# saumyarr8/ApproximateQueryEngine

Hardware: AMD Instinct MI355X
Metric: aggregates/sec (10M-row-per-GPU APPROX AVG/SUM/COUNT with 95% CI, CLT --e 0.01) + achieved HBM GB/s (higher is better)
Workload: dtype f64; 1 GPU; configs[1]: 10M-row APPROX AVG/SUM/COUNT, CLT --e 0.01 percent (never converges: full 20% dual-pointer sweep, should_stop armed), table resident in HBM; step = 100 launches x 32 different queries per launch, every result fetched; rows_per_gpu=10000000, global_rows=10000000, queries_per_launch=32, samples_per_query_per_gpu=4000000

## Files before the change

approximatequeryengine_amd/csrc/kernels.hpp:

```cpp
#pragma once

#include <hip/hip_runtime.h>

#include <cstdint>

#include "../../include/aqe_hip.h"
#include "planner.hpp"

namespace aqe {

constexpr int kBlockThreads = 256;
constexpr int kWavesPerBlock = kBlockThreads / 64;
constexpr int kTileUnroll = 8;
constexpr int kTileOrdinals = 64 * kTileUnroll;
constexpr int kDenseTileOrdinals = 2 * kTileOrdinals;
__host__ __device__ inline bool is_dense16(uint64_t step, uint32_t flags, uint64_t seg_len) { return step == 1 && !(flags & AQE_F_PAIR) && seg_len >= static_cast<uint64_t>(kTileOrdinals); }
inline uint64_t tile_ordinals(uint64_t step, uint32_t flags, uint64_t seg_len) { return is_dense16(step, flags, seg_len) ? kDenseTileOrdinals : kTileOrdinals; }
constexpr uint32_t kFamLinear = 1u << 8;
constexpr int kMaxBlocks = 2048;
constexpr unsigned kRoundGridCap = 1024;
constexpr int kVec = AQE_MOMENT_VEC;
constexpr int kShards = 64;
constexpr int kShardStride = 32;
constexpr int kCounterWords = (kShards + 1) * kShardStride;
// ... 186 lines not shown
    LeanTail tail;
    LeanRuns runs;
};
static_assert(sizeof(LeanLaunch) <= 4096, "kernel arguments are limited to 4 KB");
constexpr int kUnionMaxPieces = 512;
constexpr int kUnionMaxEntries = 768;
constexpr int kUnionMaxIncidences = 2048;
constexpr int kUnionMaxRows = 256;
constexpr int kUnionWgPieces = 32;
constexpr int kUnionJudgeSlots = 32;
constexpr int kUnionDenseWaves = 4;
constexpr int kUnionMaxTilesPerWg = 64 * kPersistWaves;
constexpr uint32_t kUnionTileWhole = 1u << 31;
struct LeanUnion {
    const uint64_t* piece_lo;
    const uint64_t* piece_hi;
    const uint32_t* piece_entry;
    const uint32_t* target_begin;
    const uint32_t* target_entry;
    uint32_t npieces, ntargets, nincidences, nentries;
    uint32_t pad[2];
};
static_assert(sizeof(LeanUnion) == 64, "the union header is staged as 8 words");
hipError_t launch_sweep_lean(const LeanLaunch& a, unsigned grid, bool nt, hipStream_t s, hipEvent_t ev0 = nullptr, hipEvent_t ev1 = nullptr);
hipError_t launch_sweep_lean_multi(const LeanLaunch* table, const unsigned long long* wg_map, unsigned long long epoch, unsigned grid, bool nt,
                                   hipStream_t s, hipEvent_t ev0 = nullptr, hipEvent_t ev1 = nullptr);

hipError_t launch_replay(const double* totals, uint32_t rounds, uint32_t has_topup, const FoldParams& fp,
                         const FinalizeParams& fin, QueryState* state, aqe_result* result, hipStream_t s);

struct ReplayItem {
    uint32_t rounds, has_topup;
    FoldParams fp;
    FinalizeParams fin;
    QueryState* state;
    aqe_result* result;
};
hipError_t launch_replay_batch(const ReplayItem* items, uint32_t n, const double* totals, uint64_t row_stride, hipStream_t s);

hipError_t launch_round(const RoundLaunch& a, hipStream_t s, hipEvent_t ev0 = nullptr, hipEvent_t ev1 = nullptr);
hipError_t launch_indexed(const RoundLaunch& a, const uint64_t* idx, uint64_t n_idx, hipStream_t s, hipEvent_t ev0 = nullptr,
                          hipEvent_t ev1 = nullptr);
hipError_t launch_permuted(const RoundLaunch& a, const PermSpec& perm, uint64_t shard_lo, uint64_t shard_rows, hipStream_t s, hipEvent_t ev0 = nullptr,
                           hipEvent_t ev1 = nullptr);
hipError_t launch_gather_permuted(const aqe_record* aos, const PermSpec& perm, aqe_record* out, hipStream_t s);
hipError_t launch_update(QueryState* state, const double* vec, const FoldParams& p, int reset_state, hipStream_t s);
hipError_t launch_finalize(const QueryState* state, const FinalizeParams& p, aqe_result* out, hipStream_t s);

hipError_t launch_gather(const aqe_record* aos, uint64_t shard_lo, const DevFamily* fams, uint32_t nfam,
// ... 49 lines not shown
```

approximatequeryengine_amd/csrc/lean.hip:

```cpp
#include <hip/hip_ext.h>

#include "device_common.hpp"

namespace aqe {
namespace {

#define AQE_RLX __ATOMIC_RELAXED, __HIP_MEMORY_SCOPE_AGENT

typedef const AQE_KARG LeanLaunch* LeanKarg;

#ifdef AQE_LEAN_STAMPS
#if AQE_LEAN_STAMPS + 0 >= 2
#define LEAN_STAMP_BLOCKS 2
#define LEAN_STAMP_BASE (static_cast<size_t>(epoch & 1ull) * kLeanStampWords)
#else
#define LEAN_STAMP_BLOCKS 1
#define LEAN_STAMP_BASE static_cast<size_t>(0)
#endif
constexpr size_t kLeanStampWords = (static_cast<size_t>(kMaxPersistGrid) * kPersistWaves + 1 + kPersistWaves) * 8;
__device__ unsigned long long g_lean_stamps[LEAN_STAMP_BLOCKS * kLeanStampWords];
#define LEAN_STAMP(slot) do { if (lane == 0 && blockIdx.x < static_cast<unsigned>(kMaxPersistGrid)) g_lean_stamps[LEAN_STAMP_BASE + (static_cast<size_t>(blockIdx.x) * kPersistWaves + wave) * 8 + (slot)] = __builtin_amdgcn_s_memrealtime(); } while (0)
#define LEAN_STAMP_FOLD(slot) do { if (threadIdx.x == 0) g_lean_stamps[LEAN_STAMP_BASE + static_cast<size_t>(kMaxPersistGrid) * kPersistWaves * 8 + (slot)] = __builtin_amdgcn_s_memrealtime(); } while (0)
#define LEAN_STAMP_JUDGE(slot) do { if (lane == 0) g_lean_stamps[LEAN_STAMP_BASE + (static_cast<size_t>(kMaxPersistGrid) * kPersistWaves + 1 + wave) * 8 + (slot)] = __builtin_amdgcn_s_memrealtime(); } while (0)
#define LEAN_STAMP_HWID(slot) do { if (lane == 0) g_lean_stamps[LEAN_STAMP_BASE + (static_cast<size_t>(kMaxPersistGrid) * kPersistWaves + 1 + wave) * 8 + (slot)] = __builtin_amdgcn_s_getreg((31 << 11) | 4); } while (0)
#else
#define LEAN_STAMP(slot) do { } while (0)
#define LEAN_STAMP_FOLD(slot) do { } while (0)
#define LEAN_STAMP_JUDGE(slot) do { } while (0)
#endif

__device__ __forceinline__ void lean_state_store(QueryState* g, const QueryState& st) {
    static_assert(sizeof(QueryState) % 8 == 0, "state is moved as 8-byte words");
    const unsigned long long* s = reinterpret_cast<const unsigned long long*>(&st);
    unsigned long long* d = reinterpret_cast<unsigned long long*>(g);
#pragma unroll
    for (unsigned i = 0; i < sizeof(QueryState) / 8; ++i) __hip_atomic_store(d + i, s[i], AQE_RLX);
}

__device__ __forceinline__ u64 read_lane_u64(u64 v, unsigned src_lane) {
    const unsigned lo = __builtin_amdgcn_readlane(static_cast<unsigned>(v), src_lane);
    const unsigned hi = __builtin_amdgcn_readlane(static_cast<unsigned>(v >> 32), src_lane);
    return (static_cast<u64>(hi) << 32) | lo;
}

__device__ __forceinline__ u64* lean_t0_word(unsigned* counter) { return reinterpret_cast<u64*>(counter + kShards * kShardStride + 8); }

struct __attribute__((packed, aligned(8))) Row2 { double x, y; };

template <bool kNT>
__device__ __forceinline__ void lean_tile(const double* base, unsigned rem, const double* safe, int lane, int has_where, double wmin, double wmax,
                                          double shift, TileAcc& ta) {
    Row2 v2[kTileUnroll];
    if (rem >= static_cast<unsigned>(kDenseTileOrdinals)) {
        const Row2* const p = reinterpret_cast<const Row2*>(base) + lane;
#pragma unroll
        for (int k = 0; k < kTileUnroll; ++k) {
            if (kNT) {
                v2[k].x = __builtin_nontemporal_load(&p[k * 64].x);
                v2[k].y = __builtin_nontemporal_load(&p[k * 64].y);
            } else {
                v2[k] = p[k * 64];
            }
        }
        ta.nv = 2u * kTileUnroll;
        if (has_where) {
#pragma unroll
            for (int k = 0; k < kTileUnroll; ++k) {
                const double x = v2[k].x, y = v2[k].y;
                const bool px = x >= wmin && x <= wmax, py = y >= wmin && y <= wmax;
                const double dx = px ? x - shift : 0.0, dy = py ? y - shift : 0.0;
// ... 214 lines not shown
            auto below = [&](double v, unsigned by) { return kW >= 16 || q >= by ? v : 0.0; };
            double p = tot[cc];
            p += below(dpp_f64<0x111>(p), 1u);
            p += below(dpp_f64<0x112>(p), 2u);
            p += below(dpp_f64<0x114>(p), 4u);
            if constexpr (kW >= 16) p += dpp_f64<0x118>(p);
            if constexpr (kW == 32) {
                const double carry = __shfl(p, static_cast<int>((static_cast<unsigned>(lane) & 32u) | 15u), 64);
                p += (lane & 16) ? carry : 0.0;
            }
            tot[cc] = p;
        }
        lean_judge<kW>(Tm, tot, static_cast<unsigned>(lane), 0ull, epoch, lds_res);
        wave_lds_handoff();
#ifdef AQE_LEAN_STAMPS
        if (m0 == wave * kPer) { LEAN_STAMP_JUDGE(0); LEAN_STAMP_HWID(2); }
#endif
        if constexpr (kW == 32) lean_send_result<32>(Tm, lds_res, static_cast<unsigned>(lane));
        else lean_send_result<kW>(*reinterpret_cast<const LeanTail*>(my_tails), results + slot0 * kLeanResWords, static_cast<unsigned>(lane));
        LEAN_STAMP_JUDGE(1);
    }
}

template <bool kNT>
__device__ __forceinline__ void lean_union(const LeanLaunch& a, const LeanUnion* const U, const LeanLaunch* const members, const unsigned nmem,
                                           const unsigned bid, const unsigned G, const unsigned long long epoch,
                                           double (&lds_part)[kMaxPersistRounds][kPersistWaves][kVec], double (&lds_round)[kMaxPersistRounds][kVec],
                                           unsigned (&lds_mask)[kPersistWaves], int& s_last) {
    static_assert(kUnionWgPieces <= kMaxPersistRounds && kUnionWgPieces <= 32, "a share's pieces: a row of lds_part and a mask bit each");
    static_assert(sizeof(LeanUnion) + sizeof(unsigned) <= sizeof(lds_round), "the union's header is staged in lds_round, the largest round count after it");
    unsigned* const lds_max_rounds = reinterpret_cast<unsigned*>(&lds_round[0][0]) + sizeof(LeanUnion) / sizeof(unsigned);
    const int lane = threadIdx.x & 63;
    const unsigned wave = threadIdx.x >> 6;
    const unsigned t_lo = bid * a.tiles_per_wg;
    const unsigned t_end = t_lo + a.tiles_per_wg < a.ntiles ? t_lo + a.tiles_per_wg : a.ntiles;
    const u64* const tile_row = reinterpret_cast<const u64*>(U + 1);
    const unsigned* const tile_meta = reinterpret_cast<const unsigned*>(tile_row + a.ntiles);
    const unsigned* const wg = tile_meta + ((a.ntiles + 1u) & ~1u) + static_cast<size_t>(bid) * (kUnionWgPieces + 1);
    const unsigned my_t = t_lo + wave + kPersistWaves * static_cast<unsigned>(lane);
    u64 my_row = 0;
    unsigned my_meta = 0;
    if (my_t < t_end) { my_row = tile_row[my_t]; my_meta = tile_meta[my_t]; }
    const unsigned p0 = __builtin_amdgcn_readfirstlane(wg[0]);
    unsigned my_entry = 0;
    if (wave == 0 && lane < kUnionWgPieces) my_entry = wg[1 + lane];
#ifdef AQE_LEAN_STAMPS
    asm volatile("s_waitcnt vmcnt(0)" ::: "memory");
    LEAN_STAMP(1);
#endif
    const bool head_stager = wave == kPersistWaves - 2u;
    u64 head_word = 0;
    if (head_stager && static_cast<unsigned>(lane) < sizeof(LeanUnion) / 8u) head_word = reinterpret_cast<const u64*>(U)[lane];
#pragma unroll
    for (unsigned i = 0; i < kMaxPersistRounds * kVec / 64; ++i) {
        const unsigned x = static_cast<unsigned>(lane) + 64u * i;
        lds_part[x >> 3][wave][x & 7u] = 0.0;
    }

    double ps = 0.0, pq = 0.0;
    unsigned pn = 0, pv = 0, cur = ~0u, touched = 0;
    auto take = [&](unsigned piece, const TileAcc& ta) {
        if (piece != cur) {
            if (cur != ~0u) {
                const double v[7] = {static_cast<double>(pn), ps, pq, static_cast<double>(pv), 0.0, 0.0, 0.0};
                const double mine = wave_sum7(v, lane);
                if ((lane & 7) == 0 && lane < 32) lds_part[cur - p0][wave][lane >> 3] = mine;
                touched |= 1u << (cur - p0);
                ps = 0.0; pq = 0.0; pn = 0; pv = 0;
            }
            cur = piece;
        }
        pn += ta.n; pv += ta.nv; ps += ta.s; pq += ta.q;
    };
    for (unsigned j = 0;; ++j) {
        if (t_lo + wave + kPersistWaves * j >= t_end) break;
        const u64 row = read_lane_u64(my_row, j);
        const unsigned meta = __builtin_amdgcn_readlane(my_meta, j), piece = meta & 0xffffu;
        const double* const base = a.amount + row;
        if (meta & kUnionTileWhole) {
            TileAcc ta;
            lean_tile<kNT>(base, static_cast<unsigned>(kDenseTileOrdinals), a.amount, lane, a.has_where, a.wmin, a.wmax, a.shift, ta);
            take(piece, ta);
#ifdef AQE_LEAN_STAMPS
            if (j == 0) LEAN_STAMP(2);
#endif
            continue;
        }
        const unsigned vhi = (meta >> 16) & 0x7ffu, vlo = (meta >> 27) & 1u;
        Row2 v2[kTileUnroll];
        bool ok[kTileUnroll];
#pragma unroll
        for (int k = 0; k < kTileUnroll; ++k) {
            const unsigned oi = 2u * static_cast<unsigned>(lane) + 128u * static_cast<unsigned>(k);
            ok[k] = oi + 1u < vhi;
            const Row2* const p = reinterpret_cast<const Row2*>(ok[k] ? base + oi : a.amount);
            if (kNT) {
                v2[k].x = __builtin_nontemporal_load(&p->x);
                v2[k].y = __builtin_nontemporal_load(&p->y);
            } else {
                v2[k] = *p;
            }
        }
        const double xo = (vhi & 1u) ? base[vhi - 1u] : 0.0;
        const u64 phi = U->piece_hi[piece];
        const bool two = phi - row < vhi;
        const unsigned mid = two ? static_cast<unsigned>(phi - row) : vhi;
        const unsigned hi = two ? (U->piece_hi[piece + 1u] - row < vhi ? static_cast<unsigned>(U->piece_hi[piece + 1u] - row) : vhi) : vhi;
        TileAcc t0, t1;
        auto add = [&](double x, unsigned r, bool ld) {
            const bool i0 = ld && r >= vlo && r < mid, i1 = ld && r >= mid && r < hi;
            const bool w = !a.has_where || (x >= a.wmin && x <= a.wmax);
            const double d0 = i0 && w ? x - a.shift : 0.0, d1 = i1 && w ? x - a.shift : 0.0;
            t0.nv += i0 ? 1u : 0u; t0.n += i0 && w ? 1u : 0u; t0.s += d0; t0.q += d0 * d0;
            t1.nv += i1 ? 1u : 0u; t1.n += i1 && w ? 1u : 0u; t1.s += d1; t1.q += d1 * d1;
        };
#pragma unroll
        for (int k = 0; k < kTileUnroll; ++k) {
            const unsigned oi = 2u * static_cast<unsigned>(lane) + 128u * static_cast<unsigned>(k);
            add(v2[k].x, oi, ok[k]);
            add(v2[k].y, oi + 1u, ok[k]);
        }
        if (vhi & 1u) add(xo, vhi - 1u, lane == 0);
        take(piece, t0);
        if (two) take(piece + 1u, t1);
#ifdef AQE_LEAN_STAMPS
        if (j == 0) LEAN_STAMP(2);
#endif
    }
    LEAN_STAMP(3);
    if (cur != ~0u) take(~0u, TileAcc{});
    if (lane == 0) lds_mask[wave] = touched;
    if (head_stager && static_cast<unsigned>(lane) < sizeof(LeanUnion) / 8u) reinterpret_cast<u64*>(&lds_round[0][0])[lane] = head_word;
    if (head_stager && lane == 0) *lds_max_rounds = 0u;
    __syncthreads();

    if (wave == 0) {
        unsigned m = 0;
#pragma unroll
        for (unsigned j = 0; j < kPersistWaves; ++j) m |= lds_mask[j];
        m = __builtin_amdgcn_readfirstlane(m);
        static_assert(kUnionWgPieces % 16 == 0, "pieces in sets of sixteen");
#pragma unroll
        for (unsigned g = 0; g < kUnionWgPieces / 16; ++g) {
            if (((m >> (16u * g)) & 0xffffu) == 0u) continue;
            const unsigned j = 16u * g + (static_cast<unsigned>(lane) >> 2), c = static_cast<unsigned>(lane) & 3u;
            const unsigned e = static_cast<unsigned>(__shfl(static_cast<int>(my_entry), static_cast<int>(j), 64));
            if ((m >> j) & 1u) {
                double x[kPersistWaves];
#pragma unroll
                for (unsigned w = 0; w < kPersistWaves; ++w) x[w] = lds_part[j][w][c];
// ... 113 lines not shown
        }
        return r;
    };
    const double r0 = tt0 < ntg ? target_sum(tb0, te0) : 0.0;
    const double r1 = tt1 < ntg ? target_sum(tb1, te1) : 0.0;
    __syncthreads();
    auto put = [&](unsigned t, double r) { rows[static_cast<size_t>(t >> 1) * 8u + (tc < 3u ? 3u * (t & 1u) + tc : 6u + (t & 1u))] = r; };
    if (tt0 < ntg) put(tt0, r0);
    if (tt1 < ntg) put(tt1, r1);
    if (i < kUnionJudgeSlots * kLeanTailWords) Ftails[i] = mt0;
    if (i + kPersistThreads < kUnionJudgeSlots * kLeanTailWords) Ftails[i + kPersistThreads] = mt1;
    __syncthreads();
    LEAN_STAMP_FOLD(5);
    static_assert(kMaxPersistRounds <= 32, "a member's rounds fit a half wave");
    const unsigned max_rounds = *lds_max_rounds;
    if (max_rounds <= 8u) lean_union_judge<8>(members, nmem, wave, lane, rows, Ftails, Fres, epoch);
    else if (max_rounds <= 16u) lean_union_judge<16>(members, nmem, wave, lane, rows, Ftails, Fres, epoch);
    else lean_union_judge<32>(members, nmem, wave, lane, rows, Ftails, Fres, epoch);
}

template <bool kNT, bool kWide>
__device__ __forceinline__ void lean_query(const LeanLaunch& a, const LeanRuns* const runs, const LeanKarg K, const LeanLaunch* const members, const unsigned nmem,
                                           const unsigned bid, const unsigned G, const unsigned long long epoch,
                                           const LeanUnion* const uni = nullptr) {
    __shared__ double lds_part[kMaxPersistRounds][kPersistWaves][kVec];
    static_assert(kMaxPersistRounds * kPersistWaves >= kLeanMaxSlots, "the partial list fits where the workgroup's own sums were");
    __shared__ double lds_round[kMaxPersistRounds][kVec];
    __shared__ unsigned lds_slot[kMaxPersistRounds];
    __shared__ unsigned lds_mask[kPersistWaves];
    __shared__ u64 lds_tail[64];
    __shared__ int s_last;
    if (uni) {
        lean_union<kNT>(a, uni, members, nmem, bid, G, epoch, lds_part, lds_round, lds_mask, s_last);
        return;
    }
    const int lane = threadIdx.x & 63;
    const unsigned wave = threadIdx.x >> 6;
    LEAN_STAMP(0);
    __shared__ u64 lds_row0[kWide ? kLeanWideRuns : 1];
    __shared__ unsigned lds_tb[kWide ? kLeanWideRuns : 1], lds_rows[kWide ? kLeanWideRuns : 1], lds_meta[kWide ? kLeanWideRuns : 1], lds_rslot[kWide ? kLeanWideRuns : 1];
    u64 my_row0 = 0, my_row0_hi = 0;
    unsigned my_tb = 0, my_rows = 0, my_meta = 0, my_slot = 0, my_tb_hi = 0, my_rows_hi = 0, my_meta_hi = 0, my_slot_hi = 0;
    if (kWide) {
        for (unsigned i = threadIdx.x; i < a.nruns; i += kPersistThreads) {
            lds_row0[i] = a.wide->row0[i]; lds_tb[i] = a.wide->tile_begin[i]; lds_rows[i] = a.wide->rows[i];
            lds_meta[i] = a.wide->meta[i]; lds_rslot[i] = a.wide->slot[i];
        }
        __syncthreads();
    } else {
        my_row0 = runs->row0[lane]; my_row0_hi = runs->row0[lane + 64];
        my_tb = runs->tile_begin[lane]; my_rows = runs->rows[lane]; my_meta = runs->meta[lane]; my_slot = runs->slot[lane];
        my_tb_hi = runs->tile_begin[lane + 64]; my_rows_hi = runs->rows[lane + 64]; my_meta_hi = runs->meta[lane + 64]; my_slot_hi = runs->slot[lane + 64];
    }
    const bool stager = wave == kPersistWaves - 1u;
    u64 tail_word = 0;
    if (stager && static_cast<unsigned>(lane) < sizeof(LeanTail) / 8u) tail_word = reinterpret_cast<const AQE_KARG u64*>(&K->tail)[lane];
// ... 199 lines not shown
#ifdef AQE_ABL_FOLD3
        if (tot[0] + tot[6] != -1.0) { if (lane == 0) T.state->n_a = tot[0] + tot[1] + tot[2] + tot[3] + tot[4] + tot[5] + tot[6]; return; }
#endif
        const LeanTail& Tm = mi == 0 ? T : *reinterpret_cast<const LeanTail*>(lds_mine);
        lean_judge(Tm, tot, static_cast<unsigned>(lane), t0, epoch, lds_res);
        wave_lds_handoff();
        lean_send_result(Tm, lds_res, static_cast<unsigned>(lane));
        mi += kPersistWaves;
        if (mi >= nmem) break;
        const u64 w = static_cast<unsigned>(lane) < kTailWords ? reinterpret_cast<const u64*>(&members[mi].tail)[lane] : 0ull;
        wave_lds_handoff();
        lds_mine[lane] = w;
        wave_lds_handoff();
    }
}

template <bool kNT, bool kWide>
__global__ __launch_bounds__(kPersistThreads) void k_sweep_lean(LeanLaunch a) {
    const LeanKarg K = (LeanKarg)__builtin_amdgcn_kernarg_segment_ptr();
    lean_query<kNT, kWide>(a, &((const LeanLaunch*)K)->runs, K, nullptr, 1u, blockIdx.x, gridDim.x, a.epoch);
}

template <bool kNT>
__global__ __launch_bounds__(kPersistThreads) void k_sweep_lean_multi(const LeanLaunch* table, const unsigned long long* wg_map, unsigned long long epoch) {
#ifdef AQE_LEAN_STAMPS
    {
        const int lane = threadIdx.x & 63;
        const unsigned wave = threadIdx.x >> 6;
        LEAN_STAMP(0);
    }
#endif
    const u64 me = uniform64(wg_map[blockIdx.x]);
    const unsigned q = static_cast<unsigned>(me >> 32) & 0xffffu, nmem = static_cast<unsigned>(me >> 48);
    const LeanKarg K = (LeanKarg)(table + q);
    LeanLaunch a;
    a.amount = K->amount; a.ntiles = K->ntiles; a.tiles_per_wg = K->tiles_per_wg;
    a.has_where = K->has_where; a.wmin = K->wmin; a.wmax = K->wmax; a.shift = K->shift;
    a.partials = K->partials; a.counter = K->counter; a.tail.want_ticks = 0; a.wide = nullptr; a.nruns = 0;
    lean_query<kNT, false>(a, &(table + q)->runs, K, table + q, nmem, static_cast<unsigned>(me) & 0xffffu, static_cast<unsigned>(me >> 16) & 0xffffu, epoch,
                           K->uni);
}

}

hipError_t launch_sweep_lean_multi(const LeanLaunch* table, const unsigned long long* wg_map, unsigned long long epoch, unsigned grid, bool nt,
                                   hipStream_t s, hipEvent_t ev0, hipEvent_t ev1) {
    if (nt) {
        if (ev0) hipExtLaunchKernelGGL(k_sweep_lean_multi<true>, dim3(grid), dim3(kPersistThreads), 0, s, ev0, ev1, 0, table, wg_map, epoch);
        else hipLaunchKernelGGL(k_sweep_lean_multi<true>, dim3(grid), dim3(kPersistThreads), 0, s, table, wg_map, epoch);
    } else {
        if (ev0) hipExtLaunchKernelGGL(k_sweep_lean_multi<false>, dim3(grid), dim3(kPersistThreads), 0, s, ev0, ev1, 0, table, wg_map, epoch);
        else hipLaunchKernelGGL(k_sweep_lean_multi<false>, dim3(grid), dim3(kPersistThreads), 0, s, table, wg_map, epoch);
    }
    return hipGetLastError();
}

hipError_t launch_sweep_lean(const LeanLaunch& a, unsigned grid, bool nt, hipStream_t s, hipEvent_t ev0, hipEvent_t ev1) {
    auto go = [&](auto kernel) {
        if (ev0) hipExtLaunchKernelGGL(kernel, dim3(grid), dim3(kPersistThreads), 0, s, ev0, ev1, 0, a);
        else hipLaunchKernelGGL(kernel, dim3(grid), dim3(kPersistThreads), 0, s, a);
    };
    if (a.wide) { if (nt) go(k_sweep_lean<true, true>); else go(k_sweep_lean<false, true>); }
    else { if (nt) go(k_sweep_lean<true, false>); else go(k_sweep_lean<false, false>); }
    return hipGetLastError();
}

#ifdef AQE_LEAN_STAMPS
extern "C" __attribute__((visibility("default"))) int aqe_debug_lean_stamps(unsigned long long* out, size_t words) {
    const size_t all = LEAN_STAMP_BLOCKS * kLeanStampWords;
    return static_cast<int>(hipMemcpyFromSymbol(out, HIP_SYMBOL(g_lean_stamps), 8 * (words < all ? words : all), 0, hipMemcpyDeviceToHost));
}
#endif

}
```

approximatequeryengine_amd/csrc/plans.hip:

```cpp
#include "host.hpp"

using namespace aqe;

namespace aqe {

void destroy_plan(aqe_plan* p, bool device_idle) {
    if (!p) return;
    if (!device_idle) (void)hipDeviceSynchronize();
    if (p->ctx && p->table_epoch == p->ctx->table_epoch) {
        if (p->view_step_rounds) release_stride_view(p->ctx, p->view_step_rounds, p->cached);
        if (p->view_step_topup) release_stride_view(p->ctx, p->view_step_topup, p->cached);
    }
    p->view_step_rounds = p->view_step_topup = 0;
    if (p->d_fams && p->d_fams != p->d_fams_small) (void)hipFree(p->d_fams);
    if (p->d_idx) (void)hipFree(p->d_idx);
    if (p->ctx && p->d_fams_small && p->partials && p->counter && p->d_state && p->h_result && p->ev0 && p->ev1 && p->d_ctl && p->d_rehearsal &&
        p->ctx->scratch_pool.size() < 128) {
        p->ctx->scratch_pool.push_back(PlanScratch{p->partials, p->counter, p->d_state, p->h_result, p->d_result, p->ev0, p->ev1, p->d_ctl, p->d_rehearsal, p->d_fams_small});
        p->partials = nullptr; p->counter = nullptr; p->d_state = nullptr; p->h_result = nullptr; p->ev0 = p->ev1 = nullptr;
        p->d_ctl = nullptr; p->d_rehearsal = nullptr; p->d_fams_small = nullptr;
    }
    if (p->partials) (void)hipFree(p->partials);
    if (p->counter) (void)hipFree(p->counter);
    if (p->d_ctl) (void)hipFree(p->d_ctl);
// ... 946 lines not shown
}

namespace {

int ensure_lanes(aqe_ctx* c) {
    while (c->lanes.size() < kBatchLanes) {
        hipStream_t s = nullptr;
        HIPCHK(c, hipStreamCreateWithFlags(&s, hipStreamNonBlocking));
        c->lanes.push_back(s);
    }
    return AQE_OK;
}

}
}

struct BatchMulti {
    bool built = false;
    std::vector<SweepForm> forms;
    PersistLaunch* d_table = nullptr;
    bool lean = false;
    LeanLaunch* d_ltable = nullptr;
    unsigned long long* d_wgmap = nullptr;
    unsigned grid = 0;
    uint64_t samples = 0;
    uint32_t classes = 0;
    uint64_t rows_loaded = 0;
    std::vector<void*> unions;
    uint64_t union_rows = 0;
    std::vector<aqe_union_shape> union_shapes;
    bool nt = false;
    const double* totals = nullptr;
    uint64_t stride = 0;
};

struct aqe_batch {
    aqe_ctx* ctx = nullptr;
    std::vector<aqe_plan*> plans;
    std::vector<hipEvent_t> swept;
    hipEvent_t reduced = nullptr;
    ReplayItem* d_items = nullptr;
    BatchMulti multi[2];
    hipStream_t last_stream = nullptr;
    int last_kind = -1;
    bool profile = false;
    bool profiled = false;
    hipEvent_t pev0 = nullptr, pev1 = nullptr;
};

namespace aqe {
namespace {

void free_multi(BatchMulti& m) {
    for (SweepForm& f : m.forms)
        if (f.d_ppart) (void)hipFree(f.d_ppart);
    m.forms.clear();
    if (m.d_table) (void)hipFree(m.d_table);
    if (m.d_ltable) (void)hipFree(m.d_ltable);
    if (m.d_wgmap) (void)hipFree(m.d_wgmap);
    for (void* u : m.unions) (void)hipFree(u);
    m.unions.clear();
    m.union_shapes.clear();
    m.d_ltable = nullptr;
    m.lean = false;
    m.d_table = nullptr;
    m.d_wgmap = nullptr;
    m.built = false;
}

void mask_member_fields(LeanLaunch& a) {
    std::memset(&a.tail.fold, 0, sizeof(a.tail.fold));
    std::memset(&a.tail.fin, 0, sizeof(a.tail.fin));
    a.tail.out_totals = nullptr; a.tail.state = nullptr; a.tail.result = nullptr; a.tail.result_seq = nullptr;
    a.partials = nullptr; a.counter = nullptr; a.epoch = 0;
}

uint64_t head_tiles(const aqe_plan* p) {
    uint64_t t = p->host.has_topup ? p->topup.ntiles : 0;
    for (size_t r = 0; r < p->r_head && r < p->rounds.size(); ++r) t += p->rounds[r].ntiles;
    return t;
}

int sweep_classes(aqe_batch* b, int kind, const std::vector<char>& head, const std::vector<uint32_t>& gs, std::vector<SweepForm>& lf,
                  std::vector<std::vector<size_t>>& classes) {
// ... 44 lines not shown
        if (!F.ok || F.wide) {
            if (F.d_ppart) (void)hipFree(F.d_ppart);
            for (size_t j = 1; j < cl.size(); ++j) alone.push_back({cl[j]});
            cl.resize(1);
            continue;
        }
        for (size_t j = 0; j < cl.size(); ++j) {
            SweepForm& f = lf[cl[j]];
            if (f.d_ppart) (void)hipFree(f.d_ppart);
            f = F;
            if (j) f.d_ppart = nullptr;
        }
    }
    classes.insert(classes.end(), alone.begin(), alone.end());
    return AQE_OK;
}

struct UnionBuilt {
    void* d_block = nullptr;
    uint32_t ntiles = 0, tiles_per_wg = 0;
    double* d_partials = nullptr;
    uint64_t slots = 0;
    std::vector<uint32_t> class_row;
    aqe_union_shape shape{};
};

int build_union(aqe_ctx* c, const std::vector<const SweepForm*>& forms, uint32_t G, UnionBuilt& out) {
    out = UnionBuilt{};
    std::vector<UnionRun> runs;
    std::map<std::vector<uint64_t>, uint32_t> seen;
    uint32_t nrows = 0;
    for (const SweepForm* F : forms) {
        std::vector<uint64_t> sig;
        for (uint32_t i = 0; i < F->nruns; ++i) { sig.push_back(F->h_runs.row0[i]); sig.push_back(F->h_runs.rows[i]); sig.push_back(F->h_runs.meta[i]); }
        sig.push_back(F->slots);
        const auto it = seen.find(sig);
        if (it != seen.end()) { out.class_row.push_back(it->second); continue; }
        seen.emplace(sig, nrows);
        out.class_row.push_back(nrows);
        for (uint32_t i = 0; i < F->nruns; ++i) {
            const uint32_t meta = F->h_runs.meta[i];
            runs.push_back(UnionRun{F->h_runs.row0[i], F->h_runs.rows[i], 2u * (nrows + (meta & 0xffu)) + ((meta & kLeanMetaGroupB) ? 1u : 0u)});
        }
        nrows += F->slots;
    }
    aqe_union_shape& sh = out.shape;
// ... 30 lines not shown
        sh.max_share_pieces = std::max(sh.max_share_pieces, pl - pf + 1u);
        if (pl - pf + 1u > static_cast<uint32_t>(kUnionWgPieces)) return declined(AQE_UNION_WG_PIECES);
        wg_first[b] = pf;
        wg_count[b] = pl - pf + 1u;
        for (uint32_t p = pf; p <= pl; ++p) piece_wgs[p].push_back(b);
    }
    std::vector<uint32_t> piece_entry(np + 1, 0);
    for (size_t p = 0; p < np; ++p) piece_entry[p + 1] = piece_entry[p] + static_cast<uint32_t>(piece_wgs[p].size());
    const uint32_t nent = piece_entry[np];
    sh.entries = nent;
    if (nent > static_cast<uint32_t>(kUnionMaxEntries)) return declined(AQE_UNION_MAX_ENTRIES);
    auto up8 = [](size_t x) { return (x + 7) & ~static_cast<size_t>(7); };
    const size_t o_row = sizeof(LeanUnion), o_meta = o_row + 8 * T, o_wg = o_meta + 4 * ((T + 1) & ~1ull);
    const size_t o_plo = up8(o_wg + 4 * static_cast<size_t>(G) * (kUnionWgPieces + 1)), o_phi = o_plo + 8 * np, o_pent = o_phi + 8 * np;
    const size_t o_tbeg = up8(o_pent + 4 * (np + 1)), o_tent = o_tbeg + 4 * static_cast<size_t>(2 * nrows + 1);
    const size_t o_part = (o_tent + 4 * ninc + 255) & ~static_cast<size_t>(255), bytes = o_part + 4 * sizeof(double) * nent;
    std::vector<uint8_t> img(bytes, 0);
    auto at = [&](size_t off) { return img.data() + off; };
    for (uint64_t t = 0; t < T; ++t) {
        const UnionTile& u = tl[t];
        const uint32_t meta = u.piece | (u.vhi << 16) | (u.vlo << 27) | (u.whole ? kUnionTileWhole : 0u);
        std::memcpy(at(o_row + 8 * t), &u.row, 8);
        std::memcpy(at(o_meta + 4 * t), &meta, 4);
    }
    for (uint32_t b = 0; b < G; ++b) {
        uint32_t rec[kUnionWgPieces + 1] = {0};
        rec[0] = wg_first[b];
        for (uint32_t j = 0; j < wg_count[b]; ++j) {
            const uint32_t p = wg_first[b] + j;
            const auto& v = piece_wgs[p];
            rec[1 + j] = piece_entry[p] + static_cast<uint32_t>(std::lower_bound(v.begin(), v.end(), b) - v.begin());
        }
        std::memcpy(at(o_wg + 4 * static_cast<size_t>(b) * (kUnionWgPieces + 1)), rec, sizeof(rec));
    }
    std::memcpy(at(o_plo), cv.piece_lo.data(), 8 * np);
    std::memcpy(at(o_phi), cv.piece_hi.data(), 8 * np);
    std::memcpy(at(o_pent), piece_entry.data(), 4 * (np + 1));
    std::memcpy(at(o_tbeg), cv.target_begin.data(), 4 * cv.target_begin.size());
    for (size_t k = 0; k < ninc; ++k) {
        const uint32_t e = piece_entry[cv.target_piece[k]];
        std::memcpy(at(o_tent + 4 * k), &e, 4);
    }
    char* d = nullptr;
    HIPCHK(c, hipMalloc(reinterpret_cast<void**>(&d), bytes));
    LeanUnion h{};
    h.piece_lo = reinterpret_cast<const uint64_t*>(d + o_plo);
// ... 195 lines not shown
        SweepForm& F = m.forms[i];
        int rc = AQE_OK;
        if (head[i]) {
            bool done = false;
            if (p->host.has_topup) {
                rc = build_sweep_form(p, true, F, g, p->r_head);
                if (rc != AQE_OK) return rc;
                if (F.step_begin[F.slots] <= static_cast<uint32_t>(kDecSteps)) done = true;
                else { (void)hipFree(F.d_ppart); F = SweepForm{}; }
            }
            if (!done) rc = build_sweep_form(p, false, F, g, p->r_head);
        } else {
            rc = build_sweep_form(p, false, F, g, R);
        }
        if (rc == AQE_OK) rc = materialize_form(c, F);
        if (rc != AQE_OK) return rc;
        fill_form(p, F, kind == 1, kind == 1 ? dev_totals + i * row_stride : nullptr, 0, false, table[i]);
        table[i].stamps = nullptr;
        table[i].want_ticks = 0;
        m.samples += F.samples;
        m.rows_loaded += F.samples;
    }
    std::vector<unsigned long long> tags;
    if (m.lean) {
        std::vector<unsigned long long> later;
        unsigned long long first = 0;
        for (size_t gi = 0; gi < groups.size(); ++gi) {
            unsigned long long g = 0, nmem = 0;
            for (size_t k : groups[gi]) {
                for (size_t i : classes[k]) g += gs[i];
                nmem += classes[k].size();
            }
            if (ublocks[gi].d_block) g = std::min<unsigned long long>(g, kMaxPersistGrid);
            const unsigned long long tag = (nmem << 48) | (first << 32) | (g << 16);
            (g % 8 == 0 ? tags : later).push_back(tag);
            first += nmem;
        }
        tags.insert(tags.end(), later.begin(), later.end());
    } else {
        for (size_t i = 0; i < n; ++i) if (gs[i] >= 8) tags.push_back((static_cast<unsigned long long>(i) << 32) | (static_cast<unsigned long long>(gs[i]) << 16));
        for (size_t i = 0; i < n; ++i) if (gs[i] < 8) tags.push_back((static_cast<unsigned long long>(i) << 32) | (static_cast<unsigned long long>(gs[i]) << 16));
    }
    for (const unsigned long long tag : tags) {
        const unsigned long long g = (tag >> 16) & 0xffffu;
        if (packed_layout) monitors.push_back(tag);
        else wgmap.push_back(tag);
        for (unsigned long long k = 1; k < g; ++k) wgmap.push_back(tag | k);
    }
    wgmap.insert(wgmap.end(), monitors.begin(), monitors.end());
    m.grid = static_cast<unsigned>(wgmap.size());
    if (m.lean) {
        HIPCHK(c, hipMalloc(reinterpret_cast<void**>(&m.d_ltable), n * sizeof(LeanLaunch)));
        HIPCHK(c, hipMemcpy(m.d_ltable, ltable.data(), n * sizeof(LeanLaunch), hipMemcpyHostToDevice));
    } else {
        HIPCHK(c, hipMalloc(reinterpret_cast<void**>(&m.d_table), n * sizeof(PersistLaunch)));
        HIPCHK(c, hipMemcpy(m.d_table, table.data(), n * sizeof(PersistLaunch), hipMemcpyHostToDevice));
    }
    HIPCHK(c, hipMalloc(reinterpret_cast<void**>(&m.d_wgmap), wgmap.size() * sizeof(unsigned long long)));
    HIPCHK(c, hipMemcpy(m.d_wgmap, wgmap.data(), wgmap.size() * sizeof(unsigned long long), hipMemcpyHostToDevice));
    {
        std::vector<std::pair<uint64_t, uint64_t>> iv;
        uint64_t sum_len = 0, swept = 0;
        for (size_t i = 0; i < n; ++i) {
            const aqe_query& q = b->plans[i]->q;
            const uint64_t lo = q.row_hi > q.row_lo ? q.row_lo : 0, hi = q.row_hi > q.row_lo ? q.row_hi : c->n_global;
            iv.emplace_back(lo, hi);
            sum_len += hi - lo;
            swept += m.forms[i].samples;
        }
        std::sort(iv.begin(), iv.end());
        uint64_t uni = 0, cur_lo = 0, cur_hi = 0;
        for (const auto& x : iv) {
            if (x.first > cur_hi) { uni += cur_hi - cur_lo; cur_lo = x.first; cur_hi = x.second; }
            else cur_hi = std::max(cur_hi, x.second);
        }
        uni += cur_hi - cur_lo;
        const double overlap = uni ? static_cast<double>(sum_len) / static_cast<double>(uni) : 1.0;
        m.nt = overlap < 1.5 && static_cast<double>(swept) * sizeof(double) / overlap > static_cast<double>(kInfinityCacheBytes);
    }
    m.totals = dev_totals;
    m.stride = row_stride;
    m.built = true;
    return AQE_OK;
}

int launch_multi(aqe_batch* b, int kind, hipStream_t s) {
    aqe_ctx* c = b->ctx;
    BatchMulti& m = b->multi[kind];
    const unsigned long long epoch = c->epoch++;
    for (size_t i = 0; i < b->plans.size(); ++i) {
        aqe_plan* p = b->plans[i];
        p->poll_epoch = kind == 0 ? epoch : 0;
        p->last_exec = kind == 0 ? 1 : 2;
        p->last_kernel = m.lean ? AQE_KERNEL_SWEEP_LEAN_MULTI : AQE_KERNEL_SWEEP_MULTI;
        p->last_first_unswept = m.forms[i].slots - m.forms[i].topup_slot;
        p->last_grid = m.forms[i].grid;
        p->lev_used = 0;
        p->timed = false;
        p->tick_timed = false;
    }
    b->profiled = b->profile;
    if (m.lean) HIPCHK(c, launch_sweep_lean_multi(m.d_ltable, m.d_wgmap, epoch, m.grid, m.nt, s, b->profile ? b->pev0 : nullptr, b->profile ? b->pev1 : nullptr));
    else HIPCHK(c, launch_sweep_multi(m.d_table, m.d_wgmap, epoch, m.grid, m.nt, s, b->profile ? b->pev0 : nullptr, b->profile ? b->pev1 : nullptr));
    b->last_stream = s;
    b->last_kind = kind;
    return AQE_OK;
}

}
}

extern "C" {

int aqe_plan_create(aqe_ctx* c, const aqe_query* q, aqe_plan** out) {
    if (!c || !q || !out) return AQE_ERR_INVALID;
    HIPCHK(c, hipSetDevice(c->device));
    return create_plan(c, q, out);
}

int aqe_plan_create_families(aqe_ctx* c, const aqe_query* q, const aqe_family* fams, uint32_t n_fams, uint64_t global_samples, int on_sorted, aqe_plan** out) {
    if (!c || !q || !out || (n_fams && !fams)) return AQE_ERR_INVALID;
    HIPCHK(c, hipSetDevice(c->device));
    aqe_query plain = *q;
    plain.row_lo = plain.row_hi = 0;
    const GivenFamilies given{fams, n_fams, global_samples, on_sorted != 0};
// ... 365 lines not shown
```

Baseline: 1.839 million aggregates/sec.

## Prefetch union tile descriptors per workgroup and software-pipeline tile loads

Builds a per-workgroup table of 16-byte tile slots (absolute address plus meta) on the host and passes it to the lean multi kernel. Each wave loads its slots at kernel entry, before reading the wg map and query table, and issues the first tile's data loads early. Inside the union loop the next tile's loads are issued after the current tile is folded, replacing the dependent chain of tile_row/tile_meta lookups. This adds a device buffer and more register pressure from holding a tile of rows across iterations.

After: 1.657 million aggregates/sec. 9.9% lower.

```diff
diff --git a/approximatequeryengine_amd/csrc/kernels.hpp b/approximatequeryengine_amd/csrc/kernels.hpp
--- a/approximatequeryengine_amd/csrc/kernels.hpp
+++ b/approximatequeryengine_amd/csrc/kernels.hpp
@@ -232,9 +232,14 @@
     uint32_t pad[2];
 };
 static_assert(sizeof(LeanUnion) == 64, "the union header is staged as 8 words");
+struct alignas(16) UnionSlot {
+    uint64_t addr;
+    uint32_t meta, pad;
+};
+static_assert(sizeof(UnionSlot) == 16, "a slot is one 16-byte load");
 hipError_t launch_sweep_lean(const LeanLaunch& a, unsigned grid, bool nt, hipStream_t s, hipEvent_t ev0 = nullptr, hipEvent_t ev1 = nullptr);
-hipError_t launch_sweep_lean_multi(const LeanLaunch* table, const unsigned long long* wg_map, unsigned long long epoch, unsigned grid, bool nt,
-                                   hipStream_t s, hipEvent_t ev0 = nullptr, hipEvent_t ev1 = nullptr);
+hipError_t launch_sweep_lean_multi(const LeanLaunch* table, const unsigned long long* wg_map, const UnionSlot* tiles, unsigned pitch,
+                                   unsigned long long epoch, unsigned grid, bool nt, hipStream_t s, hipEvent_t ev0 = nullptr, hipEvent_t ev1 = nullptr);
 
 hipError_t launch_replay(const double* totals, uint32_t rounds, uint32_t has_topup, const FoldParams& fp,
                          const FinalizeParams& fin, QueryState* state, aqe_result* result, hipStream_t s);
diff --git a/approximatequeryengine_amd/csrc/lean.hip b/approximatequeryengine_amd/csrc/lean.hip
--- a/approximatequeryengine_amd/csrc/lean.hip
+++ b/approximatequeryengine_amd/csrc/lean.hip
@@ -46,6 +46,43 @@
 __device__ __forceinline__ u64* lean_t0_word(unsigned* counter) { return reinterpret_cast<u64*>(counter + kShards * kShardStride + 8); }
 
 struct __attribute__((packed, aligned(8))) Row2 { double x, y; };
+
+template <bool kNT>
+__device__ __forceinline__ void dense_tile_load(const double* base, int lane, Row2 (&v2)[kTileUnroll]) {
+    const Row2* const p = reinterpret_cast<const Row2*>(base) + lane;
+#pragma unroll
+    for (int k = 0; k < kTileUnroll; ++k) {
+        if (kNT) {
+            v2[k].x = __builtin_nontemporal_load(&p[k * 64].x);
+            v2[k].y = __builtin_nontemporal_load(&p[k * 64].y);
+        } else {
+            v2[k] = p[k * 64];
+        }
+    }
+}
+
+__device__ __forceinline__ void dense_tile_fold(const Row2 (&v2)[kTileUnroll], int has_where, double wmin, double wmax, double shift, TileAcc& ta) {
+    ta.nv = 2u * kTileUnroll;
+    if (has_where) {
+#pragma unroll
+        for (int k = 0; k < kTileUnroll; ++k) {
+            const double x = v2[k].x, y = v2[k].y;
+            const bool px = x >= wmin && x <= wmax, py = y >= wmin && y <= wmax;
+            const double dx = px ? x - shift : 0.0, dy = py ? y - shift : 0.0;
+            ta.n += (px ? 1u : 0u) + (py ? 1u : 0u);
+            ta.s += dx; ta.q += dx * dx;
+            ta.s += dy; ta.q += dy * dy;
+        }
+    } else {
+        ta.n = 2u * kTileUnroll;
+#pragma unroll
+        for (int k = 0; k < kTileUnroll; ++k) {
+            const double dx = v2[k].x - shift, dy = v2[k].y - shift;
+            ta.s += dx; ta.q += dx * dx;
+            ta.s += dy; ta.q += dy * dy;
+        }
+    }
+}
 
 template <bool kNT>
 __device__ __forceinline__ void lean_tile(const double* base, unsigned rem, const double* safe, int lane, int has_where, double wmin, double wmax,
@@ -306,9 +343,44 @@
     }
 }
 
+struct UnionHeld {
+    u64 addr = 0;
+    unsigned meta = 0;
+    Row2 v2[kTileUnroll];
+    double xo = 0.0;
+    const double* safe = nullptr;
+};
+
+__device__ __forceinline__ const double* union_rows(u64 addr) {
+    typedef const __attribute__((address_space(1))) double* GlobalRows;
+    return (const double*)(GlobalRows)addr;
+}
+
+template <bool kNT>
+__device__ __forceinline__ void union_tile_load(const double* base, unsigned meta, int lane, UnionHeld& h) {
+    if (meta & kUnionTileWhole) {
+        dense_tile_load<kNT>(base, lane, h.v2);
+        h.xo = 0.0;
+        return;
+    }
+    const unsigned vhi = (meta >> 16) & 0x7ffu;
+#pragma unroll
+    for (int k = 0; k < kTileUnroll; ++k) {
+        const unsigned oi = 2u * static_cast<unsigned>(lane) + 128u * static_cast<unsigned>(k);
+        const Row2* const p = reinterpret_cast<const Row2*>(oi + 1u < vhi ? base + oi : h.safe);
+        if (kNT) {
+            h.v2[k].x = __builtin_nontemporal_load(&p->x);
+            h.v2[k].y = __builtin_nontemporal_load(&p->y);
+        } else {
+            h.v2[k] = *p;
+        }
+    }
+    h.xo = (vhi & 1u) ? base[vhi - 1u] : 0.0;
+}
+
 template <bool kNT>
 __device__ __forceinline__ void lean_union(const LeanLaunch& a, const LeanUnion* const U, const LeanLaunch* const members, const unsigned nmem,
-                                           const unsigned bid, const unsigned G, const unsigned long long epoch,
+                                           const unsigned bid, const unsigned G, const unsigned long long epoch, UnionHeld& held,
                                            double (&lds_part)[kMaxPersistRounds][kPersistWaves][kVec], double (&lds_round)[kMaxPersistRounds][kVec],
                                            unsigned (&lds_mask)[kPersistWaves], int& s_last) {
     static_assert(kUnionWgPieces <= kMaxPersistRounds && kUnionWgPieces <= 32, "a share's pieces: a row of lds_part and a mask bit each");
@@ -316,22 +388,11 @@
     unsigned* const lds_max_rounds = reinterpret_cast<unsigned*>(&lds_round[0][0]) + sizeof(LeanUnion) / sizeof(unsigned);
     const int lane = threadIdx.x & 63;
     const unsigned wave = threadIdx.x >> 6;
-    const unsigned t_lo = bid * a.tiles_per_wg;
-    const unsigned t_end = t_lo + a.tiles_per_wg < a.ntiles ? t_lo + a.tiles_per_wg : a.ntiles;
-    const u64* const tile_row = reinterpret_cast<const u64*>(U + 1);
-    const unsigned* const tile_meta = reinterpret_cast<const unsigned*>(tile_row + a.ntiles);
+    const unsigned* const tile_meta = reinterpret_cast<const unsigned*>(reinterpret_cast<const u64*>(U + 1) + a.ntiles);
     const unsigned* const wg = tile_meta + ((a.ntiles + 1u) & ~1u) + static_cast<size_t>(bid) * (kUnionWgPieces + 1);
-    const unsigned my_t = t_lo + wave + kPersistWaves * static_cast<unsigned>(lane);
-    u64 my_row = 0;
-    unsigned my_meta = 0;
-    if (my_t < t_end) { my_row = tile_row[my_t]; my_meta = tile_meta[my_t]; }
     const unsigned p0 = __builtin_amdgcn_readfirstlane(wg[0]);
     unsigned my_entry = 0;
     if (wave == 0 && lane < kUnionWgPieces) my_entry = wg[1 + lane];
-#ifdef AQE_LEAN_STAMPS
-    asm volatile("s_waitcnt vmcnt(0)" ::: "memory");
-    LEAN_STAMP(1);
-#endif
     const bool head_stager = wave == kPersistWaves - 2u;
     u64 head_word = 0;
     if (head_stager && static_cast<unsigned>(lane) < sizeof(LeanUnion) / 8u) head_word = reinterpret_cast<const u64*>(U)[lane];
@@ -356,60 +417,53 @@
         }
         pn += ta.n; pv += ta.nv; ps += ta.s; pq += ta.q;
     };
-    for (unsigned j = 0;; ++j) {
-        if (t_lo + wave + kPersistWaves * j >= t_end) break;
-        const u64 row = read_lane_u64(my_row, j);
-        const unsigned meta = __builtin_amdgcn_readlane(my_meta, j), piece = meta & 0xffffu;
-        const double* const base = a.amount + row;
+    u64 addr = read_lane_u64(held.addr, 0);
+    unsigned meta = __builtin_amdgcn_readlane(held.meta, 0);
+    for (unsigned j = 0; addr != 0;) {
+        const unsigned piece = meta & 0xffffu;
+        const double* const base = union_rows(addr);
+        const Row2 (&v2)[kTileUnroll] = held.v2;
         if (meta & kUnionTileWhole) {
             TileAcc ta;
-            lean_tile<kNT>(base, static_cast<unsigned>(kDenseTileOrdinals), a.amount, lane, a.has_where, a.wmin, a.wmax, a.shift, ta);
+            dense_tile_fold(v2, a.has_where, a.wmin, a.wmax, a.shift, ta);
             take(piece, ta);
-#ifdef AQE_LEAN_STAMPS
-            if (j == 0) LEAN_STAMP(2);
-#endif
-            continue;
-        }
-        const unsigned vhi = (meta >> 16) & 0x7ffu, vlo = (meta >> 27) & 1u;
-        Row2 v2[kTileUnroll];
-        bool ok[kTileUnroll];
-#pragma unroll
-        for (int k = 0; k < kTileUnroll; ++k) {
-            const unsigned oi = 2u * static_cast<unsigned>(lane) + 128u * static_cast<unsigned>(k);
-            ok[k] = oi + 1u < vhi;
-            const Row2* const p = reinterpret_cast<const Row2*>(ok[k] ? base + oi : a.amount);
-            if (kNT) {
-                v2[k].x = __builtin_nontemporal_load(&p->x);
-                v2[k].y = __builtin_nontemporal_load(&p->y);
-            } else {
-                v2[k] = *p;
-            }
-        }
-        const double xo = (vhi & 1u) ? base[vhi - 1u] : 0.0;
-        const u64 phi = U->piece_hi[piece];
-        const bool two = phi - row < vhi;
-        const unsigned mid = two ? static_cast<unsigned>(phi - row) : vhi;
-        const unsigned hi = two ? (U->piece_hi[piece + 1u] - row < vhi ? static_cast<unsigned>(U->piece_hi[piece + 1u] - row) : vhi) : vhi;
-        TileAcc t0, t1;
-        auto add = [&](double x, unsigned r, bool ld) {
-            const bool i0 = ld && r >= vlo && r < mid, i1 = ld && r >= mid && r < hi;
-            const bool w = !a.has_where || (x >= a.wmin && x <= a.wmax);
-            const double d0 = i0 && w ? x - a.shift : 0.0, d1 = i1 && w ? x - a.shift : 0.0;
-            t0.nv += i0 ? 1u : 0u; t0.n += i0 && w ? 1u : 0u; t0.s += d0; t0.q += d0 * d0;
-            t1.nv += i1 ? 1u : 0u; t1.n += i1 && w ? 1u : 0u; t1.s += d1; t1.q += d1 * d1;
-        };
-#pragma unroll
-        for (int k = 0; k < kTileUnroll; ++k) {
-            const unsigned oi = 2u * static_cast<unsigned>(lane) + 128u * static_cast<unsigned>(k);
-            add(v2[k].x, oi, ok[k]);
-            add(v2[k].y, oi + 1u, ok[k]);
-        }
-        if (vhi & 1u) add(xo, vhi - 1u, lane == 0);
-        take(piece, t0);
-        if (two) take(piece + 1u, t1);
+        } else {
+            const unsigned vhi = (meta >> 16) & 0x7ffu, vlo = (meta >> 27) & 1u;
+            const u64 row = static_cast<u64>(base - a.amount);
+            bool ok[kTileUnroll];
+#pragma unroll
+            for (int k = 0; k < kTileUnroll; ++k) ok[k] = 2u * static_cast<unsigned>(lane) + 128u * static_cast<unsigned>(k) + 1u < vhi;
+            const double xo = held.xo;
+            const u64 phi = U->piece_hi[piece];
+            const bool two = phi - row < vhi;
+            const unsigned mid = two ? static_cast<unsigned>(phi - row) : vhi;
+            const unsigned hi = two ? (U->piece_hi[piece + 1u] - row < vhi ? static_cast<unsigned>(U->piece_hi[piece + 1u] - row) : vhi) : vhi;
+            TileAcc t0, t1;
+            auto add = [&](double x, unsigned r, bool ld) {
+                const bool i0 = ld && r >= vlo && r < mid, i1 = ld && r >= mid && r < hi;
+                const bool w = !a.has_where || (x >= a.wmin && x <= a.wmax);
+                const double d0 = i0 && w ? x - a.shift : 0.0, d1 = i1 && w ? x - a.shift : 0.0;
+                t0.nv += i0 ? 1u : 0u; t0.n += i0 && w ? 1u : 0u; t0.s += d0; t0.q += d0 * d0;
+                t1.nv += i1 ? 1u : 0u; t1.n += i1 && w ? 1u : 0u; t1.s += d1; t1.q += d1 * d1;
+            };
+#pragma unroll
+            for (int k = 0; k < kTileUnroll; ++k) {
+                const unsigned oi = 2u * static_cast<unsigned>(lane) + 128u * static_cast<unsigned>(k);
+                add(v2[k].x, oi, ok[k]);
+                add(v2[k].y, oi + 1u, ok[k]);
+            }
+            if (vhi & 1u) add(xo, vhi - 1u, lane == 0);
+            take(piece, t0);
+            if (two) take(piece + 1u, t1);
+        }
 #ifdef AQE_LEAN_STAMPS
         if (j == 0) LEAN_STAMP(2);
 #endif
+        if (++j == 64u) break;
+        addr = read_lane_u64(held.addr, j);
+        if (addr == 0) break;
+        meta = __builtin_amdgcn_readlane(held.meta, j);
+        union_tile_load<kNT>(union_rows(addr), meta, lane, held);
     }
     LEAN_STAMP(3);
     if (cur != ~0u) take(~0u, TileAcc{});
@@ -569,7 +623,7 @@
 template <bool kNT, bool kWide>
 __device__ __forceinline__ void lean_query(const LeanLaunch& a, const LeanRuns* const runs, const LeanKarg K, const LeanLaunch* const members, const unsigned nmem,
                                            const unsigned bid, const unsigned G, const unsigned long long epoch,
-                                           const LeanUnion* const uni = nullptr) {
+                                           const LeanUnion* const uni = nullptr, UnionHeld* const held = nullptr) {
     __shared__ double lds_part[kMaxPersistRounds][kPersistWaves][kVec];
     static_assert(kMaxPersistRounds * kPersistWaves >= kLeanMaxSlots, "the partial list fits where the workgroup's own sums were");
     __shared__ double lds_round[kMaxPersistRounds][kVec];
@@ -578,7 +632,7 @@
     __shared__ u64 lds_tail[64];
     __shared__ int s_last;
     if (uni) {
-        lean_union<kNT>(a, uni, members, nmem, bid, G, epoch, lds_part, lds_round, lds_mask, s_last);
+        lean_union<kNT>(a, uni, members, nmem, bid, G, epoch, *held, lds_part, lds_round, lds_mask, s_last);
         return;
     }
     const int lane = threadIdx.x & 63;
@@ -824,15 +878,27 @@
 }
 
 template <bool kNT>
-__global__ __launch_bounds__(kPersistThreads) void k_sweep_lean_multi(const LeanLaunch* table, const unsigned long long* wg_map, unsigned long long epoch) {
+__global__ __launch_bounds__(kPersistThreads) void k_sweep_lean_multi(const LeanLaunch* table, const unsigned long long* wg_map, const UnionSlot* tiles, unsigned pitch,
+                                                                      unsigned long long epoch) {
+    const int lane = threadIdx.x & 63;
+    const unsigned wave = threadIdx.x >> 6;
+    LEAN_STAMP(0);
+    UnionHeld held;
+    held.safe = reinterpret_cast<const double*>(tiles);
+    if (kPersistWaves * static_cast<unsigned>(lane) < pitch) {
+        const UnionSlot s = tiles[static_cast<size_t>(blockIdx.x) * pitch + wave + kPersistWaves * static_cast<unsigned>(lane)];
+        held.addr = s.addr;
+        held.meta = s.meta;
+    }
+    const u64 me = uniform64(wg_map[blockIdx.x]);
 #ifdef AQE_LEAN_STAMPS
-    {
-        const int lane = threadIdx.x & 63;
-        const unsigned wave = threadIdx.x >> 6;
-        LEAN_STAMP(0);
-    }
-#endif
-    const u64 me = uniform64(wg_map[blockIdx.x]);
+    if (pitch) {
+        asm volatile("s_waitcnt vmcnt(0)" ::: "memory");
+        LEAN_STAMP(1);
+    }
+#endif
+    const u64 first = read_lane_u64(held.addr, 0);
+    if (first != 0) union_tile_load<kNT>(union_rows(first), __builtin_amdgcn_readlane(held.meta, 0), lane, held);
     const unsigned q = static_cast<unsigned>(me >> 32) & 0xffffu, nmem = static_cast<unsigned>(me >> 48);
     const LeanKarg K = (LeanKarg)(table + q);
     LeanLaunch a;
@@ -840,19 +906,19 @@
     a.has_where = K->has_where; a.wmin = K->wmin; a.wmax = K->wmax; a.shift = K->shift;
     a.partials = K->partials; a.counter = K->counter; a.tail.want_ticks = 0; a.wide = nullptr; a.nruns = 0;
     lean_query<kNT, false>(a, &(table + q)->runs, K, table + q, nmem, static_cast<unsigned>(me) & 0xffffu, static_cast<unsigned>(me >> 16) & 0xffffu, epoch,
-                           K->uni);
-}
-
-}
-
-hipError_t launch_sweep_lean_multi(const LeanLaunch* table, const unsigned long long* wg_map, unsigned long long epoch, unsigned grid, bool nt,
-                                   hipStream_t s, hipEvent_t ev0, hipEvent_t ev1) {
+                           K->uni, &held);
+}
+
+}
+
+hipError_t launch_sweep_lean_multi(const LeanLaunch* table, const unsigned long long* wg_map, const UnionSlot* tiles, unsigned pitch,
+                                   unsigned long long epoch, unsigned grid, bool nt, hipStream_t s, hipEvent_t ev0, hipEvent_t ev1) {
     if (nt) {
-        if (ev0) hipExtLaunchKernelGGL(k_sweep_lean_multi<true>, dim3(grid), dim3(kPersistThreads), 0, s, ev0, ev1, 0, table, wg_map, epoch);
-        else hipLaunchKernelGGL(k_sweep_lean_multi<true>, dim3(grid), dim3(kPersistThreads), 0, s, table, wg_map, epoch);
+        if (ev0) hipExtLaunchKernelGGL(k_sweep_lean_multi<true>, dim3(grid), dim3(kPersistThreads), 0, s, ev0, ev1, 0, table, wg_map, tiles, pitch, epoch);
+        else hipLaunchKernelGGL(k_sweep_lean_multi<true>, dim3(grid), dim3(kPersistThreads), 0, s, table, wg_map, tiles, pitch, epoch);
     } else {
-        if (ev0) hipExtLaunchKernelGGL(k_sweep_lean_multi<false>, dim3(grid), dim3(kPersistThreads), 0, s, ev0, ev1, 0, table, wg_map, epoch);
-        else hipLaunchKernelGGL(k_sweep_lean_multi<false>, dim3(grid), dim3(kPersistThreads), 0, s, table, wg_map, epoch);
+        if (ev0) hipExtLaunchKernelGGL(k_sweep_lean_multi<false>, dim3(grid), dim3(kPersistThreads), 0, s, ev0, ev1, 0, table, wg_map, tiles, pitch, epoch);
+        else hipLaunchKernelGGL(k_sweep_lean_multi<false>, dim3(grid), dim3(kPersistThreads), 0, s, table, wg_map, tiles, pitch, epoch);
     }
     return hipGetLastError();
 }
diff --git a/approximatequeryengine_amd/csrc/plans.hip b/approximatequeryengine_amd/csrc/plans.hip
--- a/approximatequeryengine_amd/csrc/plans.hip
+++ b/approximatequeryengine_amd/csrc/plans.hip
@@ -992,6 +992,8 @@
     bool lean = false;
     LeanLaunch* d_ltable = nullptr;
     unsigned long long* d_wgmap = nullptr;
+    UnionSlot* d_tiles = nullptr;
+    unsigned tile_pitch = 0;
     unsigned grid = 0;
     uint64_t samples = 0;
     uint32_t classes = 0;
@@ -1030,6 +1032,9 @@
     if (m.d_wgmap) (void)hipFree(m.d_wgmap);
     for (void* u : m.unions) (void)hipFree(u);
     m.unions.clear();
+    if (m.d_tiles) (void)hipFree(m.d_tiles);
+    m.d_tiles = nullptr;
+    m.tile_pitch = 0;
     m.union_shapes.clear();
     m.d_ltable = nullptr;
     m.lean = false;
@@ -1120,6 +1125,8 @@
     double* d_partials = nullptr;
     uint64_t slots = 0;
     std::vector<uint32_t> class_row;
+    std::vector<uint64_t> tile_row;
+    std::vector<uint32_t> tile_meta;
     aqe_union_shape shape{};
 };
 
@@ -1196,6 +1203,8 @@
         const uint32_t meta = u.piece | (u.vhi << 16) | (u.vlo << 27) | (u.whole ? kUnionTileWhole : 0u);
         std::memcpy(at(o_row + 8 * t), &u.row, 8);
         std::memcpy(at(o_meta + 4 * t), &meta, 4);
+        out.tile_row.push_back(u.row);
+        out.tile_meta.push_back(meta);
     }
     for (uint32_t b = 0; b < G; ++b) {
         uint32_t rec[kUnionWgPieces + 1] = {0};
@@ -1437,10 +1446,12 @@
         m.rows_loaded += F.samples;
     }
     std::vector<unsigned long long> tags;
+    std::map<unsigned long long, size_t> union_at;
     if (m.lean) {
         std::vector<unsigned long long> later;
         unsigned long long first = 0;
         for (size_t gi = 0; gi < groups.size(); ++gi) {
+            if (ublocks[gi].d_block) union_at[first] = gi;
             unsigned long long g = 0, nmem = 0;
             for (size_t k : groups[gi]) {
                 for (size_t i : classes[k]) g += gs[i];
@@ -1473,6 +1484,24 @@
     }
     HIPCHK(c, hipMalloc(reinterpret_cast<void**>(&m.d_wgmap), wgmap.size() * sizeof(unsigned long long)));
     HIPCHK(c, hipMemcpy(m.d_wgmap, wgmap.data(), wgmap.size() * sizeof(unsigned long long), hipMemcpyHostToDevice));
+    if (!union_at.empty()) {
+        uint32_t pitch = 0;
+        for (const auto& at : union_at) pitch = std::max(pitch, ublocks[at.second].tiles_per_wg);
+        pitch = (pitch + kPersistWaves - 1u) / kPersistWaves * kPersistWaves;
+        std::vector<UnionSlot> slots(wgmap.size() * static_cast<size_t>(pitch), UnionSlot{0, 0, 0});
+        for (size_t p = 0; p < wgmap.size(); ++p) {
+            const auto at = union_at.find((wgmap[p] >> 32) & 0xffffu);
+            if (at == union_at.end()) continue;
+            const UnionBuilt& u = ublocks[at->second];
+            const uintptr_t amount = reinterpret_cast<uintptr_t>(ltable[at->first].amount);
+            const uint64_t t_lo = (wgmap[p] & 0xffffu) * u.tiles_per_wg;
+            for (uint64_t i = 0; i < u.tiles_per_wg && t_lo + i < u.ntiles; ++i)
+                slots[p * pitch + i] = UnionSlot{amount + sizeof(double) * u.tile_row[t_lo + i], u.tile_meta[t_lo + i], 0};
+        }
+        HIPCHK(c, hipMalloc(reinterpret_cast<void**>(&m.d_tiles), slots.size() * sizeof(UnionSlot)));
+        HIPCHK(c, hipMemcpy(m.d_tiles, slots.data(), slots.size() * sizeof(UnionSlot), hipMemcpyHostToDevice));
+        m.tile_pitch = pitch;
+    }
     {
         std::vector<std::pair<uint64_t, uint64_t>> iv;
         uint64_t sum_len = 0, swept = 0;
@@ -1515,7 +1544,7 @@
         p->tick_timed = false;
     }
     b->profiled = b->profile;
-    if (m.lean) HIPCHK(c, launch_sweep_lean_multi(m.d_ltable, m.d_wgmap, epoch, m.grid, m.nt, s, b->profile ? b->pev0 : nullptr, b->profile ? b->pev1 : nullptr));
+    if (m.lean) HIPCHK(c, launch_sweep_lean_multi(m.d_ltable, m.d_wgmap, m.d_tiles, m.tile_pitch, epoch, m.grid, m.nt, s, b->profile ? b->pev0 : nullptr, b->profile ? b->pev1 : nullptr));
     else HIPCHK(c, launch_sweep_multi(m.d_table, m.d_wgmap, epoch, m.grid, m.nt, s, b->profile ? b->pev0 : nullptr, b->profile ? b->pev1 : nullptr));
     b->last_stream = s;
     b->last_kind = kind;
```
